# fabianschenk/REVO

Hardware: AMD Instinct MI355X
Metric: tracked frames/sec at 640x480, 4-level pyramid; ATE vs reference (higher is better)
Workload: dtype f32

## Files before the change

revo_amd/csrc/revo_track.hip:

```cpp
#include "revo_dev.h"
#include "revo_div.h"
#include "revo_track_dev.h"

namespace {

enum { MODE_EVAL = 0, MODE_COST = 1, MODE_DONE = 2 };
enum { PH_FIRST = 0, PH_LM = 1, PH_REFILL = 2, PH_EVAL_ONLY = 3 };
#define NWAVES (TRACK_THREADS / 64)
#define KMAX TRACK_KMAX
#define NVAL TRACK_NVAL
#define NSUM 40
#define SPIN_LIMIT 400000
#define MAX_TOTAL_EVALS 6000
static_assert(CSLOT + KMAX <= 32 && NVAL == 48 && NSUM == 40 && 1 + KMAX <= 8, "slot layout");
#define NVAL_X TRACK_NVAL_X
#define NSUM_X 68
static_assert(XERR + 1 + KMAX <= 32 && NVAL_X == 4 * 32 + KMAX && NSUM_X == 64 + KMAX && NVAL_X <= TRACK_MAIL_NVAL, "exact slot layout");

struct Cand {
  float R[9], T[3];
  float q[4];
  float incsq;
  float pad[3];
};
// ... 256 lines not shown
  if (lane < NVAL)
    __hip_atomic_store(&slot[member * NVAL + lane], ((u64)epoch << 32) | (u64)word, __ATOMIC_RELAXED, __HIP_MEMORY_SCOPE_AGENT);
}
template <int NC>
__device__ __forceinline__ bool cluster_poll(const u64* __restrict__ slot, int cluster, unsigned epoch, int lane, double* tot_out) {
  const bool isd = lane >= 32, odd = (lane & 1) != 0;
  const int my = lane < NVAL ? lane : 0;
  double tot = 0.0;
  if (NC > 0) {
    u64 g[NC > 0 ? NC : 1];
    for (unsigned spins = 0;; ++spins) {
      bool all = true;
#pragma unroll
      for (int j = 0; j < NC; ++j) g[j] = __hip_atomic_load(&slot[j * NVAL + my], __ATOMIC_RELAXED, __HIP_MEMORY_SCOPE_AGENT);
#pragma unroll
      for (int j = 0; j < NC; ++j) all = all && ((unsigned)(g[j] >> 32) == epoch);
      if (__all(all)) break;
      if (spins > SPIN_LIMIT) return false;
      __builtin_amdgcn_s_sleep(1);
    }
#pragma unroll
    for (int j = 0; j < NC; ++j) {
      const unsigned wd = (unsigned)g[j];
      const unsigned pw = __float_as_uint(lane_xor<1>(__uint_as_float(wd)));
      const double dd = __longlong_as_double((long long)(((u64)(odd ? wd : pw) << 32) | (u64)(odd ? pw : wd)));
      tot += isd ? dd : (double)__uint_as_float(wd);
    }
  } else {
    for (unsigned spins = 0;; ++spins) {
      bool all = true;
      for (int j = 0; j < cluster; ++j)
        all = all && ((unsigned)(__hip_atomic_load(&slot[j * NVAL + my], __ATOMIC_RELAXED, __HIP_MEMORY_SCOPE_AGENT) >> 32) == epoch);
      if (__all(all)) break;
      if (spins > SPIN_LIMIT) return false;
      __builtin_amdgcn_s_sleep(1);
    }
    for (int j = 0; j < cluster; ++j) {
      const unsigned wd = (unsigned)__hip_atomic_load(&slot[j * NVAL + my], __ATOMIC_RELAXED, __HIP_MEMORY_SCOPE_AGENT);
      const unsigned pw = __float_as_uint(lane_xor<1>(__uint_as_float(wd)));
      const double dd = __longlong_as_double((long long)(((u64)(odd ? wd : pw) << 32) | (u64)(odd ? pw : wd)));
      tot += isd ? dd : (double)__uint_as_float(wd);
    }
  }
  *tot_out = tot;
  return true;
}
__device__ __forceinline__ bool cluster_gather(const u64* __restrict__ mail_pair, int cluster, unsigned epoch, int lane,
                                               double* tot_out) {
  const u64* slot = mail_pair + (size_t)(epoch & 1u) * cluster * NVAL;
  switch (cluster) {
    case 2: return cluster_poll<2>(slot, cluster, epoch, lane, tot_out);
    case 3: return cluster_poll<3>(slot, cluster, epoch, lane, tot_out);
    case 4: return cluster_poll<4>(slot, cluster, epoch, lane, tot_out);
    case 6: return cluster_poll<6>(slot, cluster, epoch, lane, tot_out);
    case 8: return cluster_poll<8>(slot, cluster, epoch, lane, tot_out);
    case 16: return cluster_poll<16>(slot, cluster, epoch, lane, tot_out);
    case 32: return cluster_poll<32>(slot, cluster, epoch, lane, tot_out);
    default: return cluster_poll<0>(slot, cluster, epoch, lane, tot_out);
  }
}
__device__ __forceinline__ void cluster_publish_x(u64* __restrict__ mail_pair, int cluster, int member, unsigned epoch, double h,
                                                  double l, int lane) {
  u64* slot = mail_pair + (size_t)(epoch & 1u) * cluster * NVAL_X + (size_t)member * NVAL_X;
  const u64 e = (u64)epoch << 32;
  if (lane < 32) {
    const u64 hb = (u64)__double_as_longlong(h), lb = (u64)__double_as_longlong(l);
    u64* g = slot + 4 * lane;
    __hip_atomic_store(&g[0], e | (hb & 0xffffffffull), __ATOMIC_RELAXED, __HIP_MEMORY_SCOPE_AGENT);
    __hip_atomic_store(&g[1], e | (hb >> 32), __ATOMIC_RELAXED, __HIP_MEMORY_SCOPE_AGENT);
    __hip_atomic_store(&g[2], e | (lb & 0xffffffffull), __ATOMIC_RELAXED, __HIP_MEMORY_SCOPE_AGENT);
    __hip_atomic_store(&g[3], e | (lb >> 32), __ATOMIC_RELAXED, __HIP_MEMORY_SCOPE_AGENT);
  } else if (lane < 32 + KMAX) {
    __hip_atomic_store(&slot[128 + lane - 32], e | (u64)__float_as_uint((float)h), __ATOMIC_RELAXED, __HIP_MEMORY_SCOPE_AGENT);
  }
}
__device__ __forceinline__ bool cluster_gather_x(const u64* __restrict__ mail_pair, int cluster, unsigned epoch, int lane, double* h_out,
                                                 double* l_out) {
  const u64* slot = mail_pair + (size_t)(epoch & 1u) * cluster * NVAL_X;
  const bool dd = lane < 32;
  const int g0 = dd ? 4 * lane : (lane < 32 + KMAX ? 128 + lane - 32 : 128);
  const int gs = dd ? 1 : 0;
  double h = 0.0, l = 0.0;
  unsigned spins = 0;
  for (int j0 = 0; j0 < cluster; j0 += 4) {
    u64 g[4][4];
    for (;; ++spins) {
      bool all = true;
#pragma unroll
      for (int jj = 0; jj < 4; ++jj) {
        const int j = j0 + jj < cluster ? j0 + jj : cluster - 1;
        const u64* m = slot + (size_t)j * NVAL_X + g0;
#pragma unroll
        for (int k = 0; k < 4; ++k) g[jj][k] = __hip_atomic_load(&m[k * gs], __ATOMIC_RELAXED, __HIP_MEMORY_SCOPE_AGENT);
      }
#pragma unroll
      for (int jj = 0; jj < 4; ++jj)
#pragma unroll
        for (int k = 0; k < 4; ++k) all = all && ((unsigned)(g[jj][k] >> 32) == epoch);
      if (__all(all)) break;
      if (spins > SPIN_LIMIT) return false;
      __builtin_amdgcn_s_sleep(1);
    }
#pragma unroll
    for (int jj = 0; jj < 4; ++jj) {
      if (j0 + jj >= cluster) break;
      if (dd) {
        const double mh = __longlong_as_double((long long)(((u64)(unsigned)g[jj][1] << 32) | (u64)(unsigned)g[jj][0]));
        const double ml = __longlong_as_double((long long)(((u64)(unsigned)g[jj][3] << 32) | (u64)(unsigned)g[jj][2]));
        dd_add(h, l, mh, ml);
      } else {
        h += (double)__uint_as_float((unsigned)g[jj][0]);
      }
    }
  }
  *h_out = h;
  *l_out = l;
  return true;
}

__device__ __forceinline__ float cost_point(const f4v p, gf32p dtm, const float* R, const float* T, const Cam& c, float ed,
                                            bool filt) {
  const float X = ((R[0] * p.x + R[3] * p.y) + R[6] * p.z) + T[0];
  const float Y = ((R[1] * p.x + R[4] * p.y) + R[7] * p.z) + T[1];
  const float Z = ((R[2] * p.x + R[5] * p.y) + R[8] * p.z) + T[2];
  const float rz = revo_recip_refined(Z);
  const float u = revo_div_with(c.fx * X, Z, rz) + c.cx;
  const float v = revo_div_with(c.fy * Y, Z, rz) + c.cy;
  float cost = 0.0f;
  if (u >= 0 && u < (float)c.w && v >= 0 && v < (float)c.h) {
    const float r = dtm[(int)floorf(v) * c.w + (int)floorf(u)];
    if (!(r > ed && filt)) cost = r;
  }
  return cost;
}

#ifndef TRACK_MAXP
#define TRACK_MAXP 2
#endif
#ifndef TRACK_WAVES_PER_EU
#define TRACK_WAVES_PER_EU 3
#endif

__device__ __forceinline__ void load_pose(const Cand& c, float* R, float* T) {
#pragma unroll
  for (int i = 0; i < 9; ++i) R[i] = __uint_as_float(__builtin_amdgcn_readfirstlane(__float_as_uint(c.R[i])));
#pragma unroll
  for (int i = 0; i < 3; ++i) T[i] = __uint_as_float(__builtin_amdgcn_readfirstlane(__float_as_uint(c.T[i])));
}

template <int NE, bool EXACT>
__device__ __forceinline__ void fused_point(const f4v p, gf32p dtm, const float* R0, const float* T0, const float (*R)[9],
                                            const float (*T)[3], const Cam& c, float edist, bool filt, float huber, float* acc,
                                            double* ed) {
  const PtState s0 = project_point(p, R0, T0, c, true);
  PtState s[NE];
#pragma unroll
  for (int j = 0; j < NE; ++j) s[j] = project_point(p, R[j], T[j], c, true);
  const DtPatch q = load_patch(dtm, c.w, s0.ix, s0.iy);
  float g00[NE], g10[NE], g01[NE], g11[NE];
  int ddx[NE], ddy[NE];
  bool hit[NE];
#pragma unroll
  for (int j = 0; j < NE; ++j) {
    ddx[j] = s[j].ix - s0.ix;
    ddy[j] = s[j].iy - s0.iy;
    hit[j] = (ddy[j] == 0 && ddx[j] >= -1 && ddx[j] <= 1) || (ddx[j] == 0 && (ddy[j] == 1 || ddy[j] == -1));
    g00[j] = g10[j] = g01[j] = g11[j] = 0.0f;
    if (!hit[j]) {
      gf32p t = dtm + s[j].iy * c.w + s[j].ix;
      g00[j] = t[0]; g10[j] = t[1]; g01[j] = t[c.w]; g11[j] = t[c.w + 1];
    }
  }
  accumulate_point<EXACT>(s0, q, c.fx, c.fy, edist, filt, huber, acc, ed);
#pragma unroll
  for (int j = 0; j < NE; ++j) {
    float d00 = g00[j], d10 = g10[j], d01 = g01[j], d11 = g11[j];
    if (hit[j]) {
      const bool same_row = ddy[j] == 0, up = ddy[j] < 0, left = ddx[j] < 0, mid = ddx[j] == 0;
      d00 = same_row ? (left ? q.b0 : (mid ? q.b1 : q.b2)) : (up ? q.a0 : q.c1);
      d10 = same_row ? (left ? q.b1 : (mid ? q.b2 : q.b3)) : (up ? q.a1 : q.c2);
      d01 = same_row ? (left ? q.c0 : (mid ? q.c1 : q.c2)) : (up ? q.b1 : q.d0);
      d11 = same_row ? (left ? q.c1 : (mid ? q.c2 : q.c3)) : (up ? q.b2 : q.d1);
    }
    const float dxdy = s[j].dx * s[j].dy;
    const float w11 = dxdy, w01 = s[j].dy - dxdy, w10 = s[j].dx - dxdy, w00 = ((1.0f - s[j].dx) - s[j].dy) + dxdy;
    float res = ((w11 * d11 + w01 * d01) + w10 * d10) + w00 * d00;
    const bool good = s[j].valid && !(res > edist && filt);
    if (!good) res = 0.0f;
    const float wr = (res <= huber) ? 1.0f : revo_div(huber, res);
    if constexpr (EXACT) accumulate_error_x<false>(res, wr, good, ed, 2 + j, acc + 1 + j);
    else accumulate_error<false>(res, wr, good, ed + 2 + j, acc + CSLOT + 1 + j);
  }
}

template <int NE, bool EXACT>
__device__ __forceinline__ void fused_block(const Cand* cand, const f4v* preg, gf4p pts, int first, int stride, int N, gf32p dtm,
                                            const Cam& cam, float edist, bool filt, float huber, float* acc, double* ed) {
  float R0[9], T0[3], R[NE][9], T[NE][3];
  load_pose(cand[0], R0, T0);
#pragma unroll
  for (int j = 0; j < NE; ++j) load_pose(cand[1 + j], R[j], T[j]);
#pragma unroll
  for (int k = 0; k < TRACK_MAXP; ++k)
    if (first + k * stride < N) fused_point<NE, EXACT>(preg[k], dtm, R0, T0, R, T, cam, edist, filt, huber, acc, ed);
  for (int i = first + TRACK_MAXP * stride; i < N; i += stride) fused_point<NE, EXACT>(pts[i], dtm, R0, T0, R, T, cam, edist, filt, huber, acc, ed);
}

#define TRACK_WAVES_PER_EU_X 2
#define TRACK_OCC __attribute__((amdgpu_waves_per_eu(EXACT ? TRACK_WAVES_PER_EU_X : TRACK_WAVES_PER_EU, \
                                                     EXACT ? TRACK_WAVES_PER_EU_X : TRACK_WAVES_PER_EU)))
template <bool ONE, bool EXACT>
__global__ void __launch_bounds__(TRACK_THREADS) TRACK_OCC k_track(const PairDesc one, const PairDesc* __restrict__ descs,
                                                                   TrackParams prm, revo_pair_result* __restrict__ out,
                                                                   EvalOut* __restrict__ eval_out, u64* __restrict__ mail,
                                                                   int n_pairs, int cluster, unsigned epoch_base,
                                                                   unsigned* seq_ptr, unsigned seq_val, float* prof_out,
                                                                   unsigned* resident) {
  __shared__ Cand s_cand[2][KMAX];
  __shared__ PassCtl s_pass[2];
  __shared__ SolverState s_sv[KMAX];
  __shared__ double s_part[NWAVES][EXACT ? NSUM_X : NSUM];
  __shared__ int s_evals[REVO_L];
#ifdef REVO_TRACK_PROFILE
  __shared__ long long s_prof[12 + 5 * REVO_L];
#define PROF_MARK(var) const long long var = clock64()
#else
#define PROF_MARK(var)
#endif
  const int b = blockIdx.x;
  const int pair = (b / (8 * cluster)) * 8 + (b % 8);
  const int member = (b / 8) % cluster;
  if (resident && threadIdx.x == 0) __hip_atomic_fetch_add(resident, 1u, __ATOMIC_RELAXED, __HIP_MEMORY_SCOPE_AGENT);
  if (pair >= n_pairs) return;
  const PairDesc& d = ONE ? one : descs[pair];
  u64* mail_pair = mail + (size_t)pair * 2 * cluster * (EXACT ? NVAL_X : NVAL);
  const int tid = threadIdx.x, lane = tid & 63, lane_inv = lane, wave = rfl_i(tid >> 6);
  int kmax = 1;
#pragma unroll
  for (int i = 0; i < REVO_L; ++i) kmax = prm.kspec[i] > kmax ? prm.kspec[i] : kmax;
  kmax = kmax > KMAX ? KMAX : kmax;
  unsigned epoch = epoch_base;
  int cur_level = -1;
  f4v preg[TRACK_MAXP > 0 ? TRACK_MAXP : 1];
#pragma unroll
  for (int k = 0; k < TRACK_MAXP; ++k) preg[k] = f4v{0.f, 0.f, 1.f, 1.f};
  int Nl[REVO_L];
#pragma unroll
  for (int i = 0; i < REVO_L; ++i) Nl[i] = d.npts[i];
  float abv = 0.0f;

  if (wave < kmax) {
    float R0[9], T0[3];
#pragma unroll
    for (int i = 0; i < 9; ++i) R0[i] = d.R[i];
#pragma unroll
    for (int i = 0; i < 3; ++i) T0[i] = d.T[i];
    PassCtl pc{MODE_EVAL, prm.lvl_begin, 1, PH_FIRST};
    int flags = 0;
    float q0[4];
    quat_from_R(R0, q0);
    if (prm.eval_only) {
      pc.phase = PH_EVAL_ONLY;
    } else if (prm.check_init) {
      pc.mode = MODE_COST; pc.level = prm.pyr_min_lvl; pc.ncand = 2;
    } else if (!UNI(is_orthogonal(R0))) {
      flags = 2;
      pc.mode = MODE_DONE;
    }
    if (lane == 0) {
      SolverState& s = s_sv[wave];
#pragma unroll
      for (int i = 0; i < 4; ++i) s.q[i] = q0[i];
#pragma unroll
      for (int i = 0; i < 3; ++i) s.t[i] = T0[i];
      s.lastErr = __builtin_nanf("");
      s.lambda = 0.f;
      s.iteration = 0; s.incTry = 0; s.flags = flags; s.total_evals = 0;
      s.good = 0; s.bad = 0;
#pragma unroll
      for (int i = 0; i < KMAX; ++i) s.lamc[i] = 0.f;
      if (wave == 0) {
#pragma unroll
        for (int i = 0; i < REVO_L; ++i) s_evals[i] = 0;
        Cand& c0 = s_cand[0][0];
        Cand& c1 = s_cand[0][1];
        if (pc.mode == MODE_COST) {
#pragma unroll
          for (int i = 0; i < 9; ++i) { c0.R[i] = (i % 4 == 0) ? 1.0f : 0.0f; c1.R[i] = R0[i]; }
#pragma unroll
          for (int i = 0; i < 3; ++i) { c0.T[i] = 0.0f; c1.T[i] = T0[i]; }
        } else {
#pragma unroll
          for (int i = 0; i < 9; ++i) c0.R[i] = R0[i];
#pragma unroll
          for (int i = 0; i < 3; ++i) c0.T[i] = T0[i];
        }
        s_pass[0] = pc;
#ifdef REVO_TRACK_PROFILE
        for (int i = 0; i < 12 + 5 * REVO_L; ++i) s_prof[i] = 0;
#endif
      }
    }
  }
  __syncthreads();

  int p = 0;
  for (;; ++p) {
    const int pb = p & 1, nb = pb ^ 1;
    const int mode = rfl_i(s_pass[pb].mode), l = rfl_i(s_pass[pb].level), ncand = rfl_i(s_pass[pb].ncand), phase = rfl_i(s_pass[pb].phase);
    if (mode == MODE_DONE) break;
    Cam cam;
    cam.fx = prm.cam[l].fx; cam.fy = prm.cam[l].fy; cam.cx = prm.cam[l].cx; cam.cy = prm.cam[l].cy;
    cam.w = prm.cam[l].w; cam.h = prm.cam[l].h;
    cam.wlim = (float)(cam.w - 2); cam.hlim = (float)(cam.h - 2);
    gf4p pts = (gf4p)d.pts[l];
    gf32p dtm = (gf32p)d.dt[l];
    int N = Nl[0];
#pragma unroll
    for (int i = 1; i < REVO_L; ++i) N = (l == i) ? Nl[i] : N;
    const bool redundant = cluster == 1 || N <= prm.redundant_n;
    const int stride = redundant ? TRACK_THREADS : cluster * TRACK_THREADS;
    const int first = redundant ? tid : member * TRACK_THREADS + tid;
    if (!redundant) ++epoch;
#ifdef REVO_TRACK_PROFILE
    const long long tp0 = clock64();
#endif
    if (l != cur_level) {
      cur_level = l;
#pragma unroll
      for (int k = 0; k < TRACK_MAXP; ++k) {
        const int i = first + k * stride;
        preg[k] = (i < N) ? pts[i] : f4v{0.f, 0.f, 1.f, 1.f};
      }
    }
    const float edist = prm.edge_distance[l];
    const bool filt = prm.use_edge_filter != 0;
    constexpr int NACC = EXACT ? KMAX : 32, NED = EXACT ? 64 : 8;
    float acc[NACC];
    double ed[NED];
#pragma unroll
    for (int k = 0; k < NACC; ++k) acc[k] = 0.0f;
#pragma unroll
    for (int k = 0; k < NED; ++k) ed[k] = 0.0;
    if (mode == MODE_COST) {
// ... 484 lines not shown
```

revo_amd/csrc/revo_track_dev.h:

```cpp
#pragma once
#include "revo_dev.h"
#include "revo_div.h"

#define CSLOT 27
#define XERR 27

namespace {

__device__ __forceinline__ bool is_orthogonal(const float* R) {
  float n2 = 0.0f;
#pragma unroll
  for (int r = 0; r < 3; ++r)
#pragma unroll
    for (int c = 0; c < 3; ++c) {
      float v = R[r] * R[c] + R[3 + r] * R[3 + c] + R[6 + r] * R[6 + c];
      v -= (r == c) ? 1.0f : 0.0f;
      n2 += v * v;
    }
  const float det = R[0] * (R[4] * R[8] - R[7] * R[5]) - R[3] * (R[1] * R[8] - R[7] * R[2]) + R[6] * (R[1] * R[5] - R[4] * R[2]);
  return sqrtf(n2) < 1e-5f && det > 0.0f;
}

template <int MASK>
__device__ __forceinline__ float lane_xor(float v) {
  const int s = (int)__float_as_uint(v);
  int r;
  if (MASK == 1) r = __builtin_amdgcn_update_dpp(0, s, 0xB1, 0xf, 0xf, true);
  else if (MASK == 2) r = __builtin_amdgcn_update_dpp(0, s, 0x4E, 0xf, 0xf, true);
  else if (MASK == 4) {
    r = __builtin_amdgcn_update_dpp(0, s, 0x104, 0xf, 0x5, false);
    r = __builtin_amdgcn_update_dpp(r, s, 0x114, 0xf, 0xa, false);
  } else if (MASK == 8) r = __builtin_amdgcn_update_dpp(0, s, 0x128, 0xf, 0xf, true);
  else return __shfl_xor(v, MASK);
  return __uint_as_float((unsigned)r);
}

__device__ __forceinline__ int idx32(int lane) {
  return ((lane & 1) << 4) | ((lane & 2) << 2) | (lane & 4) | ((lane & 8) >> 2) | ((lane & 16) >> 4);
}

template <int MASK>
__device__ __forceinline__ double lane_xor_d(double v) {
  const unsigned long long u = (unsigned long long)__double_as_longlong(v);
  const unsigned lo = __float_as_uint(lane_xor<MASK>(__uint_as_float((unsigned)u)));
  const unsigned hi = __float_as_uint(lane_xor<MASK>(__uint_as_float((unsigned)(u >> 32))));
  return __longlong_as_double((long long)(((unsigned long long)hi << 32) | lo));
}

__device__ __forceinline__ void dd_acc(double& h, double& l, double x) {
  const double s = h + x, bb = s - h;
  l += (h - (s - bb)) + (x - bb);
  h = s;
}
__device__ __forceinline__ void dd_add(double& h, double& l, double h2, double l2) {
  const double s = h + h2, bb = s - h;
  double e = (h - (s - bb)) + (h2 - bb);
  e += l + l2;
  h = s + e;
  l = e - (h - s);
}
__device__ __forceinline__ float dd_to_float(double h, double l) {
  const double s = h + l, bb = s - h;
  const double e = (h - (s - bb)) + (l - bb);
  long long bits = __double_as_longlong(s);
  if (e != 0.0 && (bits & 1) == 0 && __builtin_isfinite(s)) bits += ((e > 0.0) == (s > 0.0)) ? 1 : -1;
  return (float)__longlong_as_double(bits);
}
template <int HALF, int MASK>
__device__ __forceinline__ void butterfly_step_x(double* h, double* l, int lane) {
  const bool up = (lane & MASK) != 0;
#pragma unroll
  for (int i = 0; i < HALF; ++i) {
    const double sh = up ? h[i] : h[HALF + i], sl = up ? l[i] : l[HALF + i];
    double kh = up ? h[HALF + i] : h[i], kl = up ? l[HALF + i] : l[i];
    dd_add(kh, kl, lane_xor_d<MASK>(sh), lane_xor_d<MASK>(sl));
    h[i] = kh; l[i] = kl;
  }
}
__device__ __forceinline__ void reduce32x(double* h, double* l, int lane) {
  butterfly_step_x<16, 1>(h, l, lane);
  butterfly_step_x<8, 2>(h, l, lane);
  butterfly_step_x<4, 4>(h, l, lane);
  butterfly_step_x<2, 8>(h, l, lane);
  butterfly_step_x<1, 16>(h, l, lane);
  dd_add(h[0], l[0], lane_xor_d<32>(h[0]), lane_xor_d<32>(l[0]));
}

typedef float f4v __attribute__((ext_vector_type(4)));
typedef const float __attribute__((address_space(1)))* gf32p;
typedef const f4v __attribute__((address_space(1)))* gf4p;

struct DtPatch { float a0, a1, b0, b1, b2, b3, c0, c1, c2, c3, d0, d1; };
typedef float f4u __attribute__((ext_vector_type(4), aligned(4)));
typedef float f2u __attribute__((ext_vector_type(2), aligned(4)));
typedef const f4u __attribute__((address_space(1)))* gf4up;
typedef const f2u __attribute__((address_space(1)))* gf2up;
__device__ __forceinline__ DtPatch load_patch(gf32p dt, int w, int ix, int iy) {
  gf32p p = dt + iy * w + ix;
  DtPatch q;
  const f2u a = *(gf2up)(p - w);
  const f4u b = *(gf4up)(p - 1);
  const f4u c = *(gf4up)(p + w - 1);
  const f2u d = *(gf2up)(p + 2 * w);
  q.a0 = a.x; q.a1 = a.y;
  q.b0 = b.x; q.b1 = b.y; q.b2 = b.z; q.b3 = b.w;
  q.c0 = c.x; q.c1 = c.y; q.c2 = c.z; q.c3 = c.w;
  q.d0 = d.x; q.d1 = d.y;
  return q;
}

struct PtState { float X, Y, Z, rz, dx, dy; int ix, iy; bool valid; };
struct Cam { float fx, fy, cx, cy, wlim, hlim; int w, h; };

__device__ __forceinline__ PtState project_point(const f4v p, const float* R, const float* T, const Cam& c, bool in_range) {
  PtState s;
  s.X = ((R[0] * p.x + R[3] * p.y) + R[6] * p.z) + T[0];
  s.Y = ((R[1] * p.x + R[4] * p.y) + R[7] * p.z) + T[1];
  s.Z = ((R[2] * p.x + R[5] * p.y) + R[8] * p.z) + T[2];
  s.rz = revo_recip_refined(s.Z);
  const float u = revo_div_with(s.X, s.Z, s.rz) * c.fx + c.cx;
  const float v = revo_div_with(s.Y, s.Z, s.rz) * c.fy + c.cy;
  s.valid = in_range && (u > 1.0f && v > 1.0f && u < c.wlim && v < c.hlim);
  s.ix = s.valid ? (int)u : 1;
  s.iy = s.valid ? (int)v : 1;
  s.dx = u - (float)s.ix;
  s.dy = v - (float)s.iy;
  if (!s.valid) { s.X = 0.0f; s.Y = 0.0f; s.Z = 1.0f; s.rz = 1.0f; s.dx = 0.0f; s.dy = 0.0f; }
  return s;
}

#define DSLOT(j) ((j) == 0 ? 0 : 1 + (j))
template <bool WITH_UNWEIGHTED>
__device__ __forceinline__ void accumulate_error(float res, float wr, bool good, double* ed, float* cnt) {
  const float r2 = res * res;
  ed[0] += (double)(wr * r2);
  if (WITH_UNWEIGHTED) ed[1] += (double)r2;
  *cnt += good ? 1.0f : 0.0f;
}
template <bool WITH_UNWEIGHTED>
__device__ __forceinline__ void accumulate_error_x(float res, float wr, bool good, double* xd, int k, float* cnt) {
  const float r2 = res * res;
  dd_acc(xd[XERR + k], xd[32 + XERR + k], (double)(r2 * wr));
  if (WITH_UNWEIGHTED) dd_acc(xd[XERR + k + 1], xd[32 + XERR + k + 1], (double)r2);
  *cnt += good ? 1.0f : 0.0f;
}

__device__ __forceinline__ void accumulate_terms_x(const PtState& s, float gx, float gy, float res, float wr, bool good, float* cnt,
                                                   double* xd) {
  const float px = s.X, py = s.Y;
  const float z = revo_div_with(1.0f, s.Z, s.rz);
  const float zs = revo_div(1.0f, s.Z * s.Z);
  float v[6];
  v[0] = z * gx;
  v[1] = z * gy;
  v[2] = (-px * zs) * gx + (-py * zs) * gy;
  v[3] = (float)((double)((-px * py * zs) * gx) + (-(1.0 + (double)(py * py * zs))) * (double)gy);
  v[4] = (float)((1.0 + (double)(px * px * zs)) * (double)gx + (double)((px * py * zs) * gy));
  v[5] = (-py * z) * gx + (px * z) * gy;
  {
    int k = 0;
#pragma unroll
    for (int a = 0; a < 6; ++a)
#pragma unroll
      for (int c = a; c < 6; ++c) { dd_acc(xd[k], xd[32 + k], (double)((v[a] * v[c]) * wr)); ++k; }
  }
  const float rw = res * wr;
#pragma unroll
  for (int a = 0; a < 6; ++a) dd_acc(xd[21 + a], xd[53 + a], (double)(v[a] * rw));
  accumulate_error_x<true>(res, wr, good, xd, 0, cnt);
}

template <bool EXACT>
__device__ __forceinline__ void accumulate_point(const PtState& s, const DtPatch& q, float fx, float fy, float edist, bool filt,
                                                 float huber, float* acc, double* ed) {
  const float gx00 = 0.5f * (q.b0 - q.b2), gy00 = 0.5f * (q.a0 - q.c1), d00 = q.b1;
  const float gx10 = 0.5f * (q.b1 - q.b3), gy10 = 0.5f * (q.a1 - q.c2), d10 = q.b2;
  const float gx01 = 0.5f * (q.c0 - q.c2), gy01 = 0.5f * (q.b1 - q.d0), d01 = q.c1;
  const float gx11 = 0.5f * (q.c1 - q.c3), gy11 = 0.5f * (q.b2 - q.d1), d11 = q.c2;
  const float dxdy = s.dx * s.dy;
  const float w11 = dxdy, w01 = s.dy - dxdy, w10 = s.dx - dxdy, w00 = ((1.0f - s.dx) - s.dy) + dxdy;
  float r0 = ((w11 * gx11 + w01 * gx01) + w10 * gx10) + w00 * gx00;
  float r1 = ((w11 * gy11 + w01 * gy01) + w10 * gy10) + w00 * gy00;
  float res = ((w11 * d11 + w01 * d01) + w10 * d10) + w00 * d00;
  const bool good = s.valid && !(res > edist && filt);
  if (!good) { r0 = 0.0f; r1 = 0.0f; res = 0.0f; }
  const float wr = (res <= huber) ? 1.0f : revo_div(huber, res);
  const float gx = fx * r0, gy = fy * r1;
  if constexpr (EXACT) {
    accumulate_terms_x(s, gx, gy, res, wr, good, acc, ed);
    return;
  }
  const float z = revo_div_with(1.0f, s.Z, s.rz);
  const float zs = z * z;
  float jv[6];
  jv[0] = z * gx;
  jv[1] = z * gy;
  jv[2] = (-s.X * zs) * gx + (-s.Y * zs) * gy;
  jv[3] = (-s.X * s.Y * zs) * gx + (-(1.0f + s.Y * s.Y * zs)) * gy;
  jv[4] = (1.0f + s.X * s.X * zs) * gx + (s.X * s.Y * zs) * gy;
  jv[5] = (-s.Y * z) * gx + (s.X * z) * gy;
  float wv[6];
#pragma unroll
  for (int a = 0; a < 6; ++a) wv[a] = wr * jv[a];
  {
    int k = 0;
#pragma unroll
    for (int a = 0; a < 6; ++a)
#pragma unroll
      for (int c = a; c < 6; ++c) { acc[k] = fmaf(wv[a], jv[c], acc[k]); ++k; }
  }
#pragma unroll
  for (int a = 0; a < 6; ++a) acc[21 + a] = fmaf(wv[a], res, acc[21 + a]);
  accumulate_error<true>(res, wr, good, ed, acc + CSLOT);
}

template <bool EXACT>
__device__ __forceinline__ void full_point(const f4v p, gf32p dtm, const float* R, const float* T, const Cam& c, float edist,
                                           bool filt, float huber, float* acc, double* ed) {
  const PtState s = project_point(p, R, T, c, true);
  const DtPatch q = load_patch(dtm, c.w, s.ix, s.iy);
  accumulate_point<EXACT>(s, q, c.fx, c.fy, edist, filt, huber, acc, ed);
}

}
```

Measured before the change: 117,400.

## Vectorize per-point tracking math with packed float2 ops

Rewrites projection, bilinear interpolation, gradient, Jacobian and normal-equation accumulation in terms of two-wide float vectors so the compiler can emit packed FP32 instructions on gfx950. The retry-candidate patch selection is also rewritten to pick whole pairs of values, and sched_barriers are placed around the main accumulation to constrain scheduling. The aim is to cut VALU instruction count per point in the hot loop. The cost is some changed FP summation order in the bilinear step, which may shift results slightly, plus possible register pressure from the vector pairs. An ISA-counting script is added for inspection.

```diff
diff --git a/profiles/track_isa_counts.py b/profiles/track_isa_counts.py
--- /dev/null
+++ b/profiles/track_isa_counts.py
@@ -0,0 +1,141 @@
+#!/usr/bin/env python3
+import argparse
+import os
+import re
+import shutil
+import subprocess
+import sys
+import tempfile
+
+ROOT = os.path.dirname(os.path.dirname(os.path.abspath(__file__)))
+FLAGS = "-O3 -std=c++17 -fPIC -ffp-contract=off -fno-fast-math -fvisibility=hidden -fvisibility-inlines-hidden -w".split()
+WAITS = ("s_waitcnt", "s_nop", "s_sleep")
+NOT_ALU = WAITS + ("s_endpgm", "s_branch", "s_cbranch", "s_setprio", "s_barrier", "s_code_end")
+UNITS = (("revo_track", "k_track"), ("revo_info", "k_pair_info"))
+ROWS = ("instructions", "VALU", "packed", "v_mov+pk_mov", "v_cndmask", "SALU", "memory")
+
+
+def unit_flags(csrc, unit):
+    m = re.search(r"^FLAGS_%s\s*=\s*(.*)$" % unit, open(os.path.join(csrc, "Makefile")).read(), re.M)
+    return m.group(1).split() if m else []
+
+
+def assembly(csrc, unit, keep=None):
+    hipcc = os.environ.get("HIPCC") or shutil.which("hipcc") or "/opt/rocm/bin/hipcc"
+    out = os.path.join(keep or tempfile.mkdtemp(prefix="track_isa_"), unit + ".s")
+    subprocess.check_call([hipcc, "--offload-arch=gfx950", "--cuda-device-only", "-S"] + FLAGS + unit_flags(csrc, unit) +
+                          ["-I", os.path.join(csrc, "..", "..", "include"), os.path.join(csrc, unit + ".hip"), "-o", out])
+    return open(out).read()
+
+
+def demangled(names):
+    filt = shutil.which("c++filt") or shutil.which("llvm-cxxfilt") or "/opt/rocm/llvm/bin/llvm-cxxfilt"
+    try:
+        out = subprocess.run([filt], input="\n".join(names), capture_output=True, text=True, check=True).stdout.split("\n")
+        return {n: re.sub(r"\(.*", "", d.replace("(anonymous namespace)::", "").replace("void ", "")) for n, d in zip(names, out)}
+    except (OSError, subprocess.CalledProcessError):
+        return {n: n for n in names}
+
+
+def tally(ops):
+    return {"instructions": len(ops),
+            "VALU": sum(o.startswith("v_") for o in ops),
+            "packed": sum(o.startswith("v_pk_") and not o.startswith("v_pk_mov") for o in ops),
+            "v_mov+pk_mov": sum(o.startswith(("v_mov", "v_pk_mov")) for o in ops),
+            "v_cndmask": sum(o.startswith("v_cndmask") for o in ops),
+            "SALU": sum(o.startswith("s_") and not o.startswith(NOT_ALU) and not o.startswith(("s_load", "s_buffer_load")) for o in ops),
+            "memory": sum(o.startswith(("global_", "flat_", "buffer_", "scratch_", "ds_", "s_load", "s_buffer_load")) for o in ops)}
+
+
+def loop_name(ops):
+    x4 = sum(o in ("global_load_dwordx4", "global_load_dwordx3") for o in ops)
+    x2 = sum(o == "global_load_dwordx2" for o in ops)
+    x1 = sum(o == "global_load_dword" for o in ops)
+    if x4 < 3:
+        return "cost pass" if x1 else "other"
+    n = (x1 + 2 * (x2 - 2)) // 4
+    return "full" if n == 0 else "full + %d retr%s" % (n, "y" if n == 1 else "ies")
+
+
+def kernels(asm, stem):
+    res = {}
+    for m in re.finditer(r"^(_Z\w*%s\w*):[^\n]*\n(.*?)^\s*\.section\s+\.rodata.*?^\s*\.amdhsa_kernel \1\n(.*?)\.end_amdhsa_kernel" % stem,
+                         asm, re.S | re.M):
+        name, body, desc = m.group(1), m.group(2), m.group(3)
+        lines = body.splitlines()
+        inner, cur, hdr = {}, None, None
+        for raw in lines:
+            blk = re.match(r"\s*\.L(BB\d+_\d+):", raw)
+            if blk or re.match(r"\s*;\s*%bb\.\d+:", raw):
+                hdr = blk.group(1) if blk else None
+            elif raw.split(";")[0].strip():
+                hdr = None
+            if "This Inner Loop Header" in raw and hdr:
+                inner[hdr] = []
+        for raw in lines:
+            ln = raw.split(";")[0].strip()
+            blk = re.match(r"\s*\.L(BB\d+_\d+):", raw)
+            if blk or re.match(r"\s*;\s*%bb\.\d+:", raw):
+                m2 = re.search(r"in Loop: Header=(BB\d+_\d+)", raw)
+                cur = m2.group(1) if m2 else (blk.group(1) if blk else None)
+                cur = cur if cur in inner else None
+            if ln and not ln.startswith(".") and not ln.endswith(":") and cur:
+                inner[cur].append(ln.split()[0])
+        loops = [(loop_name(o), tally(o)) for o in inner.values() if "global_load_dwordx4" in o]
+        rsrc = {"VGPRs allocated": (int(re.search(r"\.amdhsa_next_free_vgpr (\d+)", desc).group(1)) + 7) // 8 * 8,
+                "scratch bytes": int(re.search(r"\.amdhsa_private_segment_fixed_size (\d+)", desc).group(1))}
+        vg = re.search(r"\.set %s\.num_vgpr, (\d+)" % re.escape(name), asm)
+        rsrc["VGPRs in use"] = int(vg.group(1)) if vg else rsrc["VGPRs allocated"]
+        res[name] = (loops, rsrc)
+    return res
+
+
+def column(csrc, keep=None):
+    col = {}
+    for unit, stem in UNITS:
+        if os.path.exists(os.path.join(csrc, unit + ".hip")):
+            col.update(kernels(assembly(csrc, unit, keep), stem))
+    return col
+
+
+def main():
+    ap = argparse.ArgumentParser(description=__doc__, formatter_class=argparse.RawDescriptionHelpFormatter)
+    ap.add_argument("--rev", action="append", default=[], help="also count this commit's sources (repeatable)")
+    ap.add_argument("--keep", help="write the working tree's assembly into this directory")
+    a = ap.parse_args()
+    cols = []
+    for rev in a.rev:
+        tmp = tempfile.mkdtemp(prefix="track_isa_src_")
+        tar = subprocess.run(["git", "-C", ROOT, "archive", rev, "revo_amd/csrc", "include"], check=True, stdout=subprocess.PIPE).stdout
+        subprocess.run(["tar", "-x", "-C", tmp], input=tar, check=True)
+        cols.append((rev, column(os.path.join(tmp, "revo_amd", "csrc"))))
+        shutil.rmtree(tmp)
+    if a.keep:
+        os.makedirs(a.keep, exist_ok=True)
+    cols.append(("working tree", column(os.path.join(ROOT, "revo_amd", "csrc"), a.keep)))
+    names = sorted(set().union(*(c.keys() for _, c in cols)))
+    nice = demangled(names)
+    head = "%-34s" % "" + "".join("%14s" % n[:13] for n, _ in cols)
+    for k in names:
+        if not any(k in c and c[k][0] for _, c in cols):
+            continue
+        print("\n%s, gfx950" % nice[k])
+        print(head)
+        for key in ("VGPRs in use", "VGPRs allocated", "scratch bytes"):
+            print("  %-32s" % key + "".join("%14s" % (c[k][1][key] if k in c else "-") for _, c in cols))
+        loops = []
+        for _, c in cols:
+            loops += [n for n, _ in c.get(k, ((), 0))[0] if n not in loops]
+        for ln in loops:
+            print("  loop: %s, per point" % ln)
+            for row in ROWS:
+                vals = [dict(c[k][0]).get(ln) if k in c else None for _, c in cols]
+                line = "    %-30s" % row + "".join("%14s" % (v[row] if v else "-") for v in vals)
+                if row == "VALU" and len(vals) > 1 and vals[0] and vals[-1]:
+                    line += "   (%+.1f %%)" % (100.0 * (vals[-1][row] - vals[0][row]) / vals[0][row])
+                print(line)
+    return 0
+
+
+if __name__ == "__main__":
+    sys.exit(main())
diff --git a/revo_amd/csrc/revo_track.hip b/revo_amd/csrc/revo_track.hip
--- a/revo_amd/csrc/revo_track.hip
+++ b/revo_amd/csrc/revo_track.hip
@@ -432,44 +432,35 @@
 __device__ __forceinline__ void fused_point(const f4v p, gf32p dtm, const float* R0, const float* T0, const float (*R)[9],
                                             const float (*T)[3], const Cam& c, float edist, bool filt, float huber, float* acc,
                                             double* ed) {
-  const PtState s0 = project_point(p, R0, T0, c, true);
+  const PtState s0 = project_point(p.x, p.y, p.z, R0, T0, c, true);
   PtState s[NE];
 #pragma unroll
-  for (int j = 0; j < NE; ++j) s[j] = project_point(p, R[j], T[j], c, true);
+  for (int j = 0; j < NE; ++j) s[j] = project_point(p.x, p.y, p.z, R[j], T[j], c, true);
   const DtPatch q = load_patch(dtm, c.w, s0.ix, s0.iy);
-  float g00[NE], g10[NE], g01[NE], g11[NE];
-  int ddx[NE], ddy[NE];
+  tpx_f2 g0[NE], g1[NE];
   bool hit[NE];
 #pragma unroll
   for (int j = 0; j < NE; ++j) {
-    ddx[j] = s[j].ix - s0.ix;
-    ddy[j] = s[j].iy - s0.iy;
-    hit[j] = (ddy[j] == 0 && ddx[j] >= -1 && ddx[j] <= 1) || (ddx[j] == 0 && (ddy[j] == 1 || ddy[j] == -1));
-    g00[j] = g10[j] = g01[j] = g11[j] = 0.0f;
+    hit[j] = retry_in_patch(s[j].ix, s[j].iy, s0.ix, s0.iy);
+    g0[j] = g1[j] = tpx_any();
     if (!hit[j]) {
       gf32p t = dtm + s[j].iy * c.w + s[j].ix;
-      g00[j] = t[0]; g10[j] = t[1]; g01[j] = t[c.w]; g11[j] = t[c.w + 1];
-    }
-  }
+      g0[j] = tpx_mk(t[0], t[1]); g1[j] = tpx_mk(t[c.w], t[c.w + 1]);
+    }
+  }
+  tpx_f2 D0[NE], D1[NE];
+#pragma unroll
+  for (int j = 0; j < NE; ++j) retry_pick(q, s[j].ix, s[j].iy, s0.ix, s0.iy, D0[j], D1[j]);
+  __builtin_amdgcn_sched_barrier(0);
   accumulate_point<EXACT>(s0, q, c.fx, c.fy, edist, filt, huber, acc, ed);
+  __builtin_amdgcn_sched_barrier(0);
+#pragma unroll
+  for (int j = 0; j < NE; ++j) { D0[j] = tpx_sel(hit[j], D0[j], g0[j]); D1[j] = tpx_sel(hit[j], D1[j], g1[j]); }
 #pragma unroll
   for (int j = 0; j < NE; ++j) {
-    float d00 = g00[j], d10 = g10[j], d01 = g01[j], d11 = g11[j];
-    if (hit[j]) {
-      const bool same_row = ddy[j] == 0, up = ddy[j] < 0, left = ddx[j] < 0, mid = ddx[j] == 0;
-      d00 = same_row ? (left ? q.b0 : (mid ? q.b1 : q.b2)) : (up ? q.a0 : q.c1);
-      d10 = same_row ? (left ? q.b1 : (mid ? q.b2 : q.b3)) : (up ? q.a1 : q.c2);
-      d01 = same_row ? (left ? q.c0 : (mid ? q.c1 : q.c2)) : (up ? q.b1 : q.d0);
-      d11 = same_row ? (left ? q.c1 : (mid ? q.c2 : q.c3)) : (up ? q.b2 : q.d1);
-    }
-    const float dxdy = s[j].dx * s[j].dy;
-    const float w11 = dxdy, w01 = s[j].dy - dxdy, w10 = s[j].dx - dxdy, w00 = ((1.0f - s[j].dx) - s[j].dy) + dxdy;
-    float res = ((w11 * d11 + w01 * d01) + w10 * d10) + w00 * d00;
-    const bool good = s[j].valid && !(res > edist && filt);
-    if (!good) res = 0.0f;
-    const float wr = (res <= huber) ? 1.0f : revo_div(huber, res);
-    if constexpr (EXACT) accumulate_error_x<false>(res, wr, good, ed, 2 + j, acc + 1 + j);
-    else accumulate_error<false>(res, wr, good, ed + 2 + j, acc + CSLOT + 1 + j);
+    const RetryTerm t = retry_term(s[j], D0[j], D1[j], edist, filt, huber);
+    if constexpr (EXACT) accumulate_error_x<false>(t.res, t.wr, t.good, ed, 2 + j, acc + 1 + j);
+    else accumulate_error<false>(t.res, t.wr, t.good, ed + 2 + j, acc + CSLOT + 1 + j);
   }
 }
 
diff --git a/revo_amd/csrc/revo_track_dev.h b/revo_amd/csrc/revo_track_dev.h
--- a/revo_amd/csrc/revo_track_dev.h
+++ b/revo_amd/csrc/revo_track_dev.h
@@ -1,6 +1,7 @@
 #pragma once
 #include "revo_dev.h"
 #include "revo_div.h"
+#include "revo_track_px.h"
 
 #define CSLOT 27
 #define XERR 27
@@ -90,7 +91,6 @@
 typedef const float __attribute__((address_space(1)))* gf32p;
 typedef const f4v __attribute__((address_space(1)))* gf4p;
 
-struct DtPatch { float a0, a1, b0, b1, b2, b3, c0, c1, c2, c3, d0, d1; };
 typedef float f4u __attribute__((ext_vector_type(4), aligned(4)));
 typedef float f2u __attribute__((ext_vector_type(2), aligned(4)));
 typedef const f4u __attribute__((address_space(1)))* gf4up;
@@ -102,31 +102,11 @@
   const f4u b = *(gf4up)(p - 1);
   const f4u c = *(gf4up)(p + w - 1);
   const f2u d = *(gf2up)(p + 2 * w);
-  q.a0 = a.x; q.a1 = a.y;
-  q.b0 = b.x; q.b1 = b.y; q.b2 = b.z; q.b3 = b.w;
-  q.c0 = c.x; q.c1 = c.y; q.c2 = c.z; q.c3 = c.w;
-  q.d0 = d.x; q.d1 = d.y;
+  q.a = tpx_mk(a.x, a.y);
+  q.b01 = tpx_mk(b.x, b.y); q.b23 = tpx_mk(b.z, b.w);
+  q.c01 = tpx_mk(c.x, c.y); q.c23 = tpx_mk(c.z, c.w);
+  q.d = tpx_mk(d.x, d.y);
   return q;
-}
-
-struct PtState { float X, Y, Z, rz, dx, dy; int ix, iy; bool valid; };
-struct Cam { float fx, fy, cx, cy, wlim, hlim; int w, h; };
-
-__device__ __forceinline__ PtState project_point(const f4v p, const float* R, const float* T, const Cam& c, bool in_range) {
-  PtState s;
-  s.X = ((R[0] * p.x + R[3] * p.y) + R[6] * p.z) + T[0];
-  s.Y = ((R[1] * p.x + R[4] * p.y) + R[7] * p.z) + T[1];
-  s.Z = ((R[2] * p.x + R[5] * p.y) + R[8] * p.z) + T[2];
-  s.rz = revo_recip_refined(s.Z);
-  const float u = revo_div_with(s.X, s.Z, s.rz) * c.fx + c.cx;
-  const float v = revo_div_with(s.Y, s.Z, s.rz) * c.fy + c.cy;
-  s.valid = in_range && (u > 1.0f && v > 1.0f && u < c.wlim && v < c.hlim);
-  s.ix = s.valid ? (int)u : 1;
-  s.iy = s.valid ? (int)v : 1;
-  s.dx = u - (float)s.ix;
-  s.dy = v - (float)s.iy;
-  if (!s.valid) { s.X = 0.0f; s.Y = 0.0f; s.Z = 1.0f; s.rz = 1.0f; s.dx = 0.0f; s.dy = 0.0f; }
-  return s;
 }
 
 #define DSLOT(j) ((j) == 0 ? 0 : 1 + (j))
@@ -147,7 +127,7 @@
 
 __device__ __forceinline__ void accumulate_terms_x(const PtState& s, float gx, float gy, float res, float wr, bool good, float* cnt,
                                                    double* xd) {
-  const float px = s.X, py = s.Y;
+  const float px = s.XY.x, py = s.XY.y;
   const float z = revo_div_with(1.0f, s.Z, s.rz);
   const float zs = revo_div(1.0f, s.Z * s.Z);
   float v[6];
@@ -173,51 +153,19 @@
 template <bool EXACT>
 __device__ __forceinline__ void accumulate_point(const PtState& s, const DtPatch& q, float fx, float fy, float edist, bool filt,
                                                  float huber, float* acc, double* ed) {
-  const float gx00 = 0.5f * (q.b0 - q.b2), gy00 = 0.5f * (q.a0 - q.c1), d00 = q.b1;
-  const float gx10 = 0.5f * (q.b1 - q.b3), gy10 = 0.5f * (q.a1 - q.c2), d10 = q.b2;
-  const float gx01 = 0.5f * (q.c0 - q.c2), gy01 = 0.5f * (q.b1 - q.d0), d01 = q.c1;
-  const float gx11 = 0.5f * (q.c1 - q.c3), gy11 = 0.5f * (q.b2 - q.d1), d11 = q.c2;
-  const float dxdy = s.dx * s.dy;
-  const float w11 = dxdy, w01 = s.dy - dxdy, w10 = s.dx - dxdy, w00 = ((1.0f - s.dx) - s.dy) + dxdy;
-  float r0 = ((w11 * gx11 + w01 * gx01) + w10 * gx10) + w00 * gx00;
-  float r1 = ((w11 * gy11 + w01 * gy01) + w10 * gy10) + w00 * gy00;
-  float res = ((w11 * d11 + w01 * d01) + w10 * d10) + w00 * d00;
-  const bool good = s.valid && !(res > edist && filt);
-  if (!good) { r0 = 0.0f; r1 = 0.0f; res = 0.0f; }
-  const float wr = (res <= huber) ? 1.0f : revo_div(huber, res);
-  const float gx = fx * r0, gy = fy * r1;
+  const PtTerm t = point_term(s, q, fx, fy, edist, filt, huber);
   if constexpr (EXACT) {
-    accumulate_terms_x(s, gx, gy, res, wr, good, acc, ed);
+    accumulate_terms_x(s, t.G.x, t.G.y, t.res, t.wr, t.good, acc, ed);
     return;
   }
-  const float z = revo_div_with(1.0f, s.Z, s.rz);
-  const float zs = z * z;
-  float jv[6];
-  jv[0] = z * gx;
-  jv[1] = z * gy;
-  jv[2] = (-s.X * zs) * gx + (-s.Y * zs) * gy;
-  jv[3] = (-s.X * s.Y * zs) * gx + (-(1.0f + s.Y * s.Y * zs)) * gy;
-  jv[4] = (1.0f + s.X * s.X * zs) * gx + (s.X * s.Y * zs) * gy;
-  jv[5] = (-s.Y * z) * gx + (s.X * z) * gy;
-  float wv[6];
-#pragma unroll
-  for (int a = 0; a < 6; ++a) wv[a] = wr * jv[a];
-  {
-    int k = 0;
-#pragma unroll
-    for (int a = 0; a < 6; ++a)
-#pragma unroll
-      for (int c = a; c < 6; ++c) { acc[k] = fmaf(wv[a], jv[c], acc[k]); ++k; }
-  }
-#pragma unroll
-  for (int a = 0; a < 6; ++a) acc[21 + a] = fmaf(wv[a], res, acc[21 + a]);
-  accumulate_error<true>(res, wr, good, ed, acc + CSLOT);
+  accumulate_normal(jacobian(s, t.G), t.wr, t.res, acc);
+  accumulate_error<true>(t.res, t.wr, t.good, ed, acc + CSLOT);
 }
 
 template <bool EXACT>
 __device__ __forceinline__ void full_point(const f4v p, gf32p dtm, const float* R, const float* T, const Cam& c, float edist,
                                            bool filt, float huber, float* acc, double* ed) {
-  const PtState s = project_point(p, R, T, c, true);
+  const PtState s = project_point(p.x, p.y, p.z, R, T, c, true);
   const DtPatch q = load_patch(dtm, c.w, s.ix, s.iy);
   accumulate_point<EXACT>(s, q, c.fx, c.fy, edist, filt, huber, acc, ed);
 }
diff --git a/revo_amd/csrc/revo_track_px.h b/revo_amd/csrc/revo_track_px.h
--- /dev/null
+++ b/revo_amd/csrc/revo_track_px.h
@@ -0,0 +1,174 @@
+#pragma once
+#include <math.h>
+
+#if defined(__HIPCC__) || defined(__CUDACC__)
+#define TPX_HD __host__ __device__ __forceinline__
+#else
+#define TPX_HD inline
+#endif
+
+namespace {
+
+#if defined(__HIP_DEVICE_COMPILE__)
+typedef float tpx_f2 __attribute__((ext_vector_type(2)));
+TPX_HD tpx_f2 tpx_mk(float a, float b) { return tpx_f2{a, b}; }
+TPX_HD tpx_f2 tpx_swap(tpx_f2 v) { return __builtin_shufflevector(v, v, 1, 0); }
+TPX_HD tpx_f2 tpx_hi_lo(tpx_f2 a, tpx_f2 b) { return __builtin_shufflevector(a, b, 1, 2); }
+TPX_HD tpx_f2 tpx_fma(tpx_f2 a, tpx_f2 b, tpx_f2 c) { return __builtin_elementwise_fma(a, b, c); }
+TPX_HD float tpx_rcp(float d) { return __builtin_amdgcn_rcpf(d); }
+TPX_HD float tpx_scalar(float v) { asm("" : "+v"(v)); return v; }
+TPX_HD tpx_f2 tpx_any() { tpx_f2 v; return __builtin_nondeterministic_value(v); }
+#else
+struct tpx_f2 { float x, y; };
+TPX_HD tpx_f2 tpx_mk(float a, float b) { return tpx_f2{a, b}; }
+TPX_HD tpx_f2 operator+(tpx_f2 a, tpx_f2 b) { return tpx_f2{a.x + b.x, a.y + b.y}; }
+TPX_HD tpx_f2 operator-(tpx_f2 a, tpx_f2 b) { return tpx_f2{a.x - b.x, a.y - b.y}; }
+TPX_HD tpx_f2 operator*(tpx_f2 a, tpx_f2 b) { return tpx_f2{a.x * b.x, a.y * b.y}; }
+TPX_HD tpx_f2 operator-(tpx_f2 a) { return tpx_f2{-a.x, -a.y}; }
+TPX_HD tpx_f2 tpx_swap(tpx_f2 v) { return tpx_f2{v.y, v.x}; }
+TPX_HD tpx_f2 tpx_hi_lo(tpx_f2 a, tpx_f2 b) { return tpx_f2{a.y, b.x}; }
+TPX_HD tpx_f2 tpx_fma(tpx_f2 a, tpx_f2 b, tpx_f2 c) { return tpx_f2{fmaf(a.x, b.x, c.x), fmaf(a.y, b.y, c.y)}; }
+TPX_HD float tpx_scalar(float v) { return v; }
+TPX_HD tpx_f2 tpx_any() { return tpx_f2{0.0f, 0.0f}; }
+TPX_HD float tpx_rcp(float d) { return 1.0f / d; }
+#endif
+TPX_HD tpx_f2 tpx_splat(float a) { return tpx_mk(a, a); }
+TPX_HD tpx_f2 tpx_sel(bool c, tpx_f2 a, tpx_f2 b) { return c ? a : b; }
+
+TPX_HD float tpx_recip_refined(float d) {
+  const float r0 = tpx_rcp(d);
+  const float e0 = fmaf(-d, r0, 1.0f);
+  return fmaf(e0, r0, r0);
+}
+TPX_HD float tpx_div_with(float n, float d, float r1) {
+  const float q0 = n * r1;
+  const float e1 = fmaf(-d, q0, n);
+  const float q1 = fmaf(e1, r1, q0);
+  const float e2 = fmaf(-d, q1, n);
+  return fmaf(e2, r1, q1);
+}
+TPX_HD float tpx_div(float n, float d) { return tpx_div_with(n, d, tpx_recip_refined(d)); }
+TPX_HD tpx_f2 tpx_div_with2(tpx_f2 n, float d, float r1) {
+  const tpx_f2 md = tpx_splat(-d), r = tpx_splat(r1);
+  const tpx_f2 q0 = n * r;
+  const tpx_f2 e1 = tpx_fma(md, q0, n);
+  const tpx_f2 q1 = tpx_fma(e1, r, q0);
+  const tpx_f2 e2 = tpx_fma(md, q1, n);
+  return tpx_fma(e2, r, q1);
+}
+
+struct Cam { float fx, fy, cx, cy, wlim, hlim; int w, h; };
+struct PtState { tpx_f2 XY; float Z, rz; tpx_f2 d; int ix, iy; bool valid; };
+struct DtPatch { tpx_f2 a, b01, b23, c01, c23, d; };
+
+TPX_HD PtState project_point(float px, float py, float pz, const float* R, const float* T, const Cam& c, bool in_range) {
+  PtState s;
+  const tpx_f2 XY = ((tpx_mk(R[0], R[1]) * tpx_splat(px) + tpx_mk(R[3], R[4]) * tpx_splat(py)) + tpx_mk(R[6], R[7]) * tpx_splat(pz)) +
+                    tpx_mk(T[0], T[1]);
+  const float Z = ((R[2] * px + R[5] * py) + R[8] * pz) + T[2];
+  const float rz = tpx_recip_refined(Z);
+  const tpx_f2 uv = tpx_div_with2(XY, Z, rz) * tpx_mk(c.fx, c.fy) + tpx_mk(c.cx, c.cy);
+  s.valid = in_range && (uv.x > 1.0f && uv.y > 1.0f && uv.x < c.wlim && uv.y < c.hlim);
+  const tpx_f2 t = tpx_sel(s.valid, uv, tpx_splat(1.0f));
+  s.ix = (int)t.x;
+  s.iy = (int)t.y;
+  s.d = t - tpx_mk((float)s.ix, (float)s.iy);
+  s.XY = tpx_sel(s.valid, XY, tpx_splat(0.0f));
+  s.Z = s.valid ? Z : 1.0f;
+  s.rz = s.valid ? rz : 1.0f;
+  return s;
+}
+
+struct BiW { tpx_f2 W0, W1; };
+TPX_HD BiW bilinear_weights(tpx_f2 d) {
+  const float dx = tpx_scalar(d.x), dy = tpx_scalar(d.y);
+  const float dxdy = dx * dy;
+  BiW w;
+  w.W0 = tpx_mk(((1.0f - dx) - dy) + dxdy, dx - dxdy);
+  w.W1 = tpx_mk(dy - dxdy, dxdy);
+  return w;
+}
+TPX_HD float bilinear(const BiW& w, tpx_f2 G0, tpx_f2 G1) {
+  const tpx_f2 P0 = w.W0 * G0, P1 = w.W1 * G1;
+  return ((P1.y + P1.x) + P0.y) + P0.x;
+}
+
+struct PtTerm { float r0, r1, res, wr; tpx_f2 G; bool good; };
+TPX_HD PtTerm point_term(const PtState& s, const DtPatch& q, float fx, float fy, float edist, bool filt, float huber) {
+  const tpx_f2 b12 = tpx_hi_lo(q.b01, q.b23), c12 = tpx_hi_lo(q.c01, q.c23), h = tpx_splat(0.5f);
+  const tpx_f2 GX0 = h * (q.b01 - q.b23), GX1 = h * (q.c01 - q.c23);
+  const tpx_f2 GY0 = h * (q.a - c12), GY1 = h * (b12 - q.d);
+  const BiW w = bilinear_weights(s.d);
+  PtTerm t;
+  t.r0 = bilinear(w, GX0, GX1);
+  t.r1 = bilinear(w, GY0, GY1);
+  t.res = bilinear(w, b12, c12);
+  t.good = s.valid && !(t.res > edist && filt);
+  if (!t.good) { t.r0 = 0.0f; t.r1 = 0.0f; t.res = 0.0f; }
+  t.wr = (t.res <= huber) ? 1.0f : tpx_div(huber, t.res);
+  t.G = tpx_mk(fx, fy) * tpx_mk(t.r0, t.r1);
+  return t;
+}
+
+struct Jac { tpx_f2 J01, J23, J45; };
+TPX_HD Jac jacobian(const PtState& s, tpx_f2 G) {
+  const float z = tpx_div_with(1.0f, s.Z, s.rz);
+  const float zs = z * z;
+  Jac j;
+  j.J01 = tpx_splat(z) * G;
+  const tpx_f2 B = ((-s.XY) * tpx_splat(zs)) * G;
+  const tpx_f2 O = tpx_splat(1.0f) + (s.XY * s.XY) * tpx_splat(zs);
+  const float xyz = (s.XY.x * s.XY.y) * zs;
+  const tpx_f2 P = tpx_splat(xyz) * G, U = O * G;
+  const tpx_f2 C = tpx_swap(s.XY * tpx_splat(z)) * G;
+  j.J23 = tpx_mk(B.x + B.y, (-P.x) + (-U.y));
+  j.J45 = tpx_mk(U.x + P.y, (-C.x) + C.y);
+  return j;
+}
+
+TPX_HD void fma_pair(float* acc, int k, tpx_f2 a, tpx_f2 b) {
+  const tpx_f2 r = tpx_fma(a, b, tpx_mk(acc[k], acc[k + 1]));
+  acc[k] = r.x;
+  acc[k + 1] = r.y;
+}
+TPX_HD void accumulate_normal(const Jac& j, float wr, float res, float* acc) {
+  const tpx_f2 wq = tpx_splat(wr);
+  const tpx_f2 W01 = wq * j.J01, W23 = wq * j.J23, W45 = wq * j.J45;
+  fma_pair(acc, 0, tpx_splat(W01.x), j.J01);
+  fma_pair(acc, 2, tpx_splat(W01.x), j.J23);
+  fma_pair(acc, 4, tpx_splat(W01.x), j.J45);
+  acc[6] = fmaf(W01.y, j.J01.y, acc[6]);
+  fma_pair(acc, 7, tpx_splat(W01.y), j.J23);
+  fma_pair(acc, 9, tpx_splat(W01.y), j.J45);
+  fma_pair(acc, 11, tpx_splat(W23.x), j.J23);
+  fma_pair(acc, 13, tpx_splat(W23.x), j.J45);
+  acc[15] = fmaf(W23.y, j.J23.y, acc[15]);
+  fma_pair(acc, 16, tpx_splat(W23.y), j.J45);
+  fma_pair(acc, 18, tpx_splat(W45.x), j.J45);
+  acc[20] = fmaf(W45.y, j.J45.y, acc[20]);
+  const tpx_f2 rq = tpx_splat(res);
+  fma_pair(acc, 21, W01, rq);
+  fma_pair(acc, 23, W23, rq);
+  fma_pair(acc, 25, W45, rq);
+}
+
+struct RetryTerm { float res, wr; bool good; };
+TPX_HD RetryTerm retry_term(const PtState& s, tpx_f2 D0, tpx_f2 D1, float edist, bool filt, float huber) {
+  RetryTerm t;
+  t.res = bilinear(bilinear_weights(s.d), D0, D1);
+  t.good = s.valid && !(t.res > edist && filt);
+  if (!t.good) t.res = 0.0f;
+  t.wr = (t.res <= huber) ? 1.0f : tpx_div(huber, t.res);
+  return t;
+}
+TPX_HD bool retry_in_patch(int ix, int iy, int ix0, int iy0) {
+  return (iy == iy0 && (unsigned)(ix - ix0 + 1) <= 2u) || (ix == ix0 && (unsigned)(iy - iy0 + 1) <= 2u);
+}
+TPX_HD void retry_pick(const DtPatch& q, int ix, int iy, int ix0, int iy0, tpx_f2& D0, tpx_f2& D1) {
+  const bool same_row = iy == iy0, up = iy < iy0, left = ix < ix0, mid = ix == ix0;
+  const tpx_f2 b12 = tpx_hi_lo(q.b01, q.b23), c12 = tpx_hi_lo(q.c01, q.c23);
+  D0 = tpx_sel(same_row, tpx_sel(left, q.b01, tpx_sel(mid, b12, q.b23)), tpx_sel(up, q.a, c12));
+  D1 = tpx_sel(same_row, tpx_sel(left, q.c01, tpx_sel(mid, c12, q.c23)), tpx_sel(up, b12, q.d));
+}
+
+}
```

Result: faster. 119,300 (median of 6 runs) (+1.7%).
